# UnaryPlus/raytrace

Measured on AMD Instinct MI355X. Metric: Msamples/s (pixels×spp/s) + achieved HBM GB/s, Cornell-box 600×600, higher is better.
Workload: dtype f64; 1 GPU; cornell 600x600 200spp depth 50; width=600, height=600, spp=200, max_depth=50, parallelism=rows interleaved over 1 GPU(s), row_block 1

## Files before the change

raytrace_amd/csrc/rt_api.hip:

```cpp
#include <hip/hip_runtime.h>

#include <algorithm>
#include <chrono>
#include <cstdarg>
#include <cstdio>
#include <cstdlib>
#include <cstring>
#include <memory>
#include <mutex>
#include <string>
#include <thread>
#include <vector>

#include "../../include/rt.h"
#include "rt_denoise.h"
#include "rt_film.h"
#include "rt_internal.h"
#include "rt_kernel_class.h"

namespace {

thread_local std::string g_err;

int fail(int code, const char* fmt, ...) __attribute__((format(printf, 2, 3)));
// ... 200 lines not shown
  auto t0 = Clock::now();
  HIP_TRY(hipSetDevice(s->device));
  DevArrays<R>& A = s->arrays<R>();
  int rc = A.upload(s->host->arrays<R>(), s->nodes, s->perlin_perm);
  if (rc) {
    A.release();
    A = DevArrays<R>();
    return rc;
  }
  A.lds_nodes = 0;
  if ((s->variant & RT_VAR_BASE) != RT_VAR_FLAT) {
    const KernelClass c = rt_class_of(sizeof(R) == 8, s->variant);
    const int waves = std::max(1, rt_class_waves(sizeof(R) == 8, c));
    const int block = rt_class_block(sizeof(R) == 8, c);
    const int per_cu = std::max(1, 4 * waves * 64 / block);
    const int budget = (163840 / per_cu / 1024) * 1024 - 1024;
    const int used = (int)rt_class_lds_bytes(sizeof(R) == 8, c, s->stack_depth, 0);
    A.lds_nodes = std::max(0, std::min(s->host->surface_nodes, (budget - used) / 64));
    if (const char* e = rt_knob("RT_AMD_LDS_NODES")) A.lds_nodes = std::min(A.lds_nodes, std::max(0, atoi(e)));
  }
  A.resident_blocks = rt_render_resident_blocks((const KernelParamsT<R>*)nullptr, s->device, s->stack_depth,
                                                s->variant, A.lds_nodes);
  if (A.resident_blocks <= 0) {
    A.release();
    A = DevArrays<R>();
    return fail(RT_E_HIP, "occupancy query failed");
  }
  s->have<R>() = true;
  s->upload_ms += ms_since(t0);
  return RT_OK;
}

struct RenderCall {
  void* d_out = nullptr;
  char* ws = nullptr;
  size_t ws_cap = 0;
  int frame_rows = 0;
  bool lone = false, resolve = true;
  int sample0 = 0;
};

template <class R>
int render_async(const rt_device_scene* s, const rt_camera_settings* cs, uint64_t seed, const rt_exec* ex,
                 const RenderCall& c, void* hip_stream) {
  if (int rc = ensure_precision<R>(s)) return rc;
  const DevArrays<R>& A = s->arrays<R>();
  constexpr bool f64 = sizeof(R) == 8;
  LaunchInputs L;
  L.resident_lanes = (long long)A.resident_blocks * rt_class_block(f64, rt_class_of(f64, s->variant));
  L.lds_nodes = A.lds_nodes;
  L.lone = c.lone || (ex && (ex->flags & RT_EXEC_SOLO));
  L.sample0 = c.sample0;
  L.out_frame_rows = c.frame_rows;
  if (const char* e = rt_knob("RT_AMD_POOL_SHIFT")) L.pool_shift = std::max(4, std::min(10, atoi(e)));
  KernelParamsT<R> P;
  std::string err;
  int rc = rt_host_render_params(*s->host, s->variant, A.rec, cs, seed, ex, L, P, err);
  if (rc) return fail(rc, "%s", err.c_str());
  P.status = s->status;
  P.out = (R*)c.d_out;
  HIP_TRY(hipSetDevice(s->device));
  const Workspace W = workspace_layout((size_t)P.tile_rows * P.cam.width, RT_ACC_WORDS(R));
  hipStream_t st = (hipStream_t)hip_stream;
  char* ws = c.ws && c.ws_cap >= W.bytes ? c.ws : nullptr;
  const bool own = ws == nullptr;
  if (own) HIP_TRY(hipMallocAsync((void**)&ws, W.bytes, st));
  HIP_TRY(hipMemsetAsync(ws, 0, W.bytes, st));
  P.accum = (unsigned long long*)ws;
  P.nanflag = (unsigned int*)(ws + W.off_flag);
  P.counter = (int*)(ws + W.off_ctr);
  rc = RT_OK;
  int reserve = A.resident_blocks > 16 * RT_GRID_RESERVE ? RT_GRID_RESERVE : 0;
  if (const char* e = rt_knob("RT_AMD_GRID_RESERVE")) reserve = std::max(0, std::min(A.resident_blocks - 1, atoi(e)));
  if (rt_launch_render(P, A.resident_blocks - reserve, s->variant, hip_stream) ||
      (c.resolve && rt_launch_resolve(P, hip_stream)))
    rc = fail(RT_E_HIP, "kernel launch failed: %s", hipGetErrorString(hipGetLastError()));
  if (own) HIP_TRY(hipFreeAsync(ws, st));
  return rc;
}

int render_any(const rt_device_scene* s, const rt_camera_settings* cs, uint64_t seed, const rt_exec* ex, bool f32,
               const RenderCall& c, void* hip_stream) {
  return f32 ? render_async<float>(s, cs, seed, ex, c, hip_stream) : render_async<double>(s, cs, seed, ex, c, hip_stream);
}

int check_flags(const rt_exec* ex) {
  const int known = RT_EXEC_F32 | RT_EXEC_ENCODE8_SRGB | RT_EXEC_ENCODE8_SQRT | RT_EXEC_SOLO;
  if (ex->flags & ~known) return fail(RT_E_INVALID, "unknown rt_exec.flags bits 0x%x", ex->flags & ~known);
  if ((ex->flags & RT_EXEC_ENCODE8_SRGB) && (ex->flags & RT_EXEC_ENCODE8_SQRT))
    return fail(RT_E_INVALID, "rt_exec.flags: RT_EXEC_ENCODE8_SRGB and RT_EXEC_ENCODE8_SQRT are exclusive");
  return RT_OK;
}

int validate_frame(const rt_camera_settings* cs, uint64_t seed, const rt_exec* ex) {
  const int h = rt_host_image_height(cs);
  if (h <= 0 || cs->image_width <= 0) return fail(RT_E_INVALID, "image %dx%d must be non-empty", cs->image_width, h);
  if (rt_host_shard_rows(h, ex) < 0) return fail(RT_E_INVALID, "invalid rt_exec");
  if (int rc = check_flags(ex)) return rc;
  KernelParams P;
  std::string err;
  if (int rc = rt_host_make_params(cs, seed, ex, P, err)) return fail(rc, "%s", err.c_str());
  return RT_OK;
}

int exec_encoding(const rt_exec* ex) {
  if (!ex) return -1;
// ... 1136 lines not shown
```

raytrace_amd/csrc/rt_build.cpp:

```cpp
#include <algorithm>
#include <cmath>
#include <cstdarg>
#include <cstdio>
#include <cstdlib>
#include <cstring>
#include <optional>
#include <utility>

#include "../../include/rt.h"
#include "rt_bvh.h"
#include "rt_encode8_table.h"
#include "rt_internal.h"
#include "rt_kernel_class.h"

const char* rt_knob(const char* name) {
  const char* on = std::getenv("RT_AMD_EXPERIMENTS");
  if (!on || !*on || std::atoi(on) == 0) return nullptr;
  return std::getenv(name);
}

namespace {

struct d3 {
  double x, y, z;
// ... 1035 lines not shown
  const DevTargetT<R>& T = P.targets[0];
  for (int k = S.first; k < S.end_quad; ++k) {
    const R* f = A.flat_recs.data() + 16 * (size_t)k;
    if (std::memcmp(f, T.n, 3 * sizeof(R)) || std::memcmp(f + 4, T.q, 3 * sizeof(R)) ||
        std::memcmp(f + 8, T.wa, 3 * sizeof(R)) || std::memcmp(f + 12, T.wb, 3 * sizeof(R)))
      continue;
    int kf, slot;
    std::memcpy(&kf, f + 3, 4);
    std::memcpy(&slot, f + 11, 4);
    if (kf != 1 || slot < 0 || slot >= (int)A.prim_shade.size()) continue;
    if (A.prim_shade[slot].kind >= 2) continue;
    P.target_defer = 1;
    P.target_rec = k;
    return 1;
  }
  return 0;
}

template <class R>
SceneRecordsT<R> rt_host_records(const HostScene& H) {
  const HostArraysT<R>& A = H.arrays<R>();
  SceneRecordsT<R> r;
  r.nodes = H.nodes.data(), r.perlin_perm = H.perlin_perm.data();
  r.prims = A.prims.data(), r.prim_uv = A.prim_uv.data(), r.motions = A.motions.data();
  r.uvframes = A.uvframes.data(), r.texels = A.texels.data(), r.perlin_grad = A.perlin_grad.data();
  r.flat_recs = A.flat_recs.data(), r.prim_shade = A.prim_shade.data(), r.mats = A.mats.data();
  r.texs = A.texs.data(), r.boxes = A.boxes.data(), r.instances = A.instances.data();
  return r;
}

template <class R>
int rt_host_render_params(const HostScene& H, int variant, const SceneRecordsT<R>& r, const rt_camera_settings* cs,
                          uint64_t seed, const rt_exec* ex, const LaunchInputs& L, KernelParamsT<R>& P,
                          std::string& err) {
  constexpr bool f64 = sizeof(R) == 8;
  const bool flat = (variant & RT_VAR_BASE) == RT_VAR_FLAT;
  std::memset(&P, 0, sizeof P);
  if (int rc = rt_host_make_params(cs, seed, ex, P, err)) return rc;
  P.nodes = r.nodes, P.perlin_perm = r.perlin_perm;
  P.prims = r.prims, P.prim_uv = r.prim_uv, P.motions = r.motions, P.uvframes = r.uvframes, P.texels = r.texels;
  P.perlin_grad = r.perlin_grad, P.flat_recs = r.flat_recs, P.prim_shade = r.prim_shade, P.mats = r.mats;
  P.texs = r.texs, P.boxes = r.boxes, P.instances = r.instances;
  P.surface_root = H.surface_root;
  P.leaf_exit_pct = f64 ? H.leaf_exit_pct64 : H.leaf_exit_pct;
  P.surface_prefix = !flat && H.n_nodes > 0 ? 1 : 0;
  P.n_media = H.n_media;
  for (int k = 0; k < H.n_media; ++k) P.media[k] = H.arrays<R>().media[k];
  for (int k = 0; k <= RT_MAX_MEDIA; ++k) P.flat_sets[k] = H.flat_sets[k];
  P.stack_depth = rt_host_stack_depth(H);
  P.lds_nodes = L.lds_nodes;
  P.n_prims = H.n_prims;
  P.pool_shift = L.pool_shift ? L.pool_shift : L.lone && flat ? 6 : 0;
  rt_host_plan_work(P, L.resident_lanes, flat, L.lone);
  P.trav_exit_pct = f64 ? H.trav_exit_pct64 : H.trav_exit_pct;
  P.out_frame_rows = L.out_frame_rows;
  P.sample0 = L.sample0;
  rt_host_match_target(H, variant, P);
  return RT_OK;
}
#define RT_INSTANTIATE(R)                                                                                           \
  template int rt_host_match_target<R>(const HostScene&, int, KernelParamsT<R>&);                                   \
  template SceneRecordsT<R> rt_host_records<R>(const HostScene&);                                                   \
  template int rt_host_render_params<R>(const HostScene&, int, const SceneRecordsT<R>&, const rt_camera_settings*, \
                                        uint64_t, const rt_exec*, const LaunchInputs&, KernelParamsT<R>&, std::string&);
RT_INSTANTIATE(float)
RT_INSTANTIATE(double)
#undef RT_INSTANTIATE

bool rt_host_media_late(const HostScene& H) {
  if (H.n_media == 0) return false;
  for (int m = 0; m < H.n_media; ++m) {
    const DevMediumT<double>& M = H.f64.media[m];
    if (!M.alias_surface && !(M.root < 0 && M.root != RT_EMPTY_ROOT)) return false;
  }
  return true;
}

FastDiv rt_host_fastdiv(uint32_t d) {
  FastDiv f{0u, 0, d, 0};
  if (d <= 1) return f;
  int l = 0;
  while ((1ull << l) < d) ++l;
  f.m = (uint32_t)((((1ull << 32) * ((1ull << l) - d)) / d) + 1);
  f.s = l - 1;
  return f;
}

template <class R>
void rt_host_plan_work(KernelParamsT<R>& P, long long resident_lanes, bool two_sizes, bool lone) {
  P.div_width = rt_host_fastdiv((uint32_t)P.cam.width);
  P.div_block = rt_host_fastdiv((uint32_t)P.row_block);
  const bool pool_given = P.pool_shift >= 4;
  if (!pool_given) P.pool_shift = __builtin_ctz(RT_POOL);
  P.trav_exit_pct = 50;
  const long long tile_pixels = (long long)P.tile_rows * P.cam.width;
  const int spp = P.cam.spp;
  const int small = two_sizes ? 3 : 4;
  int chunk = spp < small ? spp : small;
  if (resident_lanes > 0 && (long long)P.tile_rows * P.cam.width * spp / 16 >= 64 * resident_lanes) chunk = 16;
  if (const char* env = rt_knob("RT_AMD_CHUNK")) {
    int c = std::atoi(env);
    if (c > 0) chunk = c;
  }
  int big = lone ? RT_BIG_CHUNK_MAX : RT_BIG_CHUNK_MAX_ASYNC, n_big = 0;
  if (const char* env = rt_knob("RT_AMD_BIG_CHUNK")) big = std::max(1, std::atoi(env));
  int tail_items = !lone ? RT_TAIL_ITEMS_ASYNC : sizeof(R) == 8 ? RT_TAIL_ITEMS_F64 : RT_TAIL_ITEMS_F32;
  if (const char* env = rt_knob("RT_AMD_TAIL_ITEMS")) tail_items = std::atoi(env);
  if (two_sizes && chunk < big && tail_items > 0 && resident_lanes > 0 && tile_pixels > 0) {
    long long t = ((long long)tail_items * chunk * resident_lanes + tile_pixels - 1) / tile_pixels;
    if (const char* env = rt_knob("RT_AMD_TAIL_SAMPLES")) t = std::max(0, std::atoi(env));
    const long long tail = ((t + chunk - 1) / chunk) * chunk;
    if (tail < spp) {
      const long long bulk = spp - tail;
      auto split = [&](int cap) {
        n_big = (int)((bulk + cap - 1) / cap);
        big = (int)((bulk + n_big - 1) / n_big);
        big = std::min(big, spp / n_big);
      };
      split(big);
      const double per_lane = (double)spp * (double)tile_pixels / (double)resident_lanes;
      for (int pass = 0; pass < 2 && !lone; ++pass) {
        const int pool_items = (pool_given ? 1 << P.pool_shift : big >= 32 ? 64 : RT_POOL) / 64;
        const int cap = (int)(0.9 * per_lane / pool_items);
        if (cap >= 1 && big > cap) split(cap);
      }
      if (big <= chunk) n_big = 0;
    }
  }
  const int n_chunks = (spp - n_big * big + chunk - 1) / chunk;
  long long items = (long long)(n_big + n_chunks) * tile_pixels;
  if (items > 0x7fffff00LL) {
    n_big = 0;
    chunk = (int)((long long)spp * tile_pixels / 0x7fffff00LL) + 1;
    items = (long long)((spp + chunk - 1) / chunk) * tile_pixels;
  }
  P.chunk = chunk;
  P.n_chunks = (spp - n_big * big + chunk - 1) / chunk;
  P.big_chunk = big;
  P.n_big_chunks = n_big;
  P.big_items = (int)((long long)n_big * tile_pixels);
  P.small_start = n_big * big;
  if (!pool_given && !lone && n_big > 0 && big >= 32) P.pool_shift = 6;
  P.div_big = rt_host_fastdiv((uint32_t)std::max(1, n_big));
  P.div_small = rt_host_fastdiv((uint32_t)std::max(1, P.n_chunks));
  P.n_items = (int)items;
  const KernelClass c{two_sizes ? RT_VAR_FLAT : RT_VAR_BVH, 0, P.n_media > 0 ? 1 : 0, false, false, 0, false};
  const int slot_pix = rt_class_agg_pix(sizeof(R) == 8, c);
  const int pool = 1 << P.pool_shift;
  auto spans = [&](int n) { return n > 0 && (pool - 1 + n - 1) / n + 1 <= slot_pix; };
  bool agg = tile_pixels < (1ll << 24);
  if (const char* env = rt_knob("RT_AMD_AGG")) agg = agg && std::atoi(env) != 0;
  P.agg_big = agg && spans(n_big);
  P.agg_small = agg && spans(P.n_chunks);
}

template int rt_host_make_params<float>(const rt_camera_settings*, uint64_t, const rt_exec*, KernelParamsT<float>&,
                                        std::string&);
template int rt_host_make_params<double>(const rt_camera_settings*, uint64_t, const rt_exec*, KernelParamsT<double>&,
                                         std::string&);
template void rt_host_plan_work<float>(KernelParamsT<float>&, long long, bool, bool);
template void rt_host_plan_work<double>(KernelParamsT<double>&, long long, bool, bool);

void rt_host_encode8_thresholds(int encoding, double* thr) {
  const double* t = encoding == 1 ? kEnc8Sqrt : kEnc8Srgb;
  for (int k = 0; k < 256; ++k) thr[k] = t[k];
}
```

raytrace_amd/csrc/rt_internal.h:

```cpp
#pragma once
#include <stdint.h>

#include <string>
#include <vector>

#ifndef RT_BLOCK
#define RT_BLOCK 64
#endif
#ifndef RT_BLOCK_BVH
#define RT_BLOCK_BVH 256
#endif
#define RT_MAX_NODES (1 << 26)
#define RT_STACK_DEPTH 64
#define RT_MAX_MEDIA 8
#define RT_MAX_TARGETS 8
#ifndef RT_LEAF_MAX
#define RT_LEAF_MAX 8
#endif
#ifndef RT_POOL
#define RT_POOL 128
#endif
#ifndef RT_AGG_SLOTS_FLAT
#define RT_AGG_SLOTS_FLAT 8
#endif
#ifndef RT_AGG_PIX_FLAT
#define RT_AGG_PIX_FLAT 17
#endif
#ifndef RT_AGG_SLOTS_FLAT_F64
#define RT_AGG_SLOTS_FLAT_F64 7
#endif
#ifndef RT_AGG_PIX_FLAT_F64
#define RT_AGG_PIX_FLAT_F64 22
#endif
#ifndef RT_AGG_SLOTS_BVH
#define RT_AGG_SLOTS_BVH 4
#endif
#ifndef RT_AGG_PIX_BVH
#define RT_AGG_PIX_BVH 5
#endif
#ifndef RT_BIG_CHUNK_MAX
#define RT_BIG_CHUNK_MAX 16
#endif
#ifndef RT_BIG_CHUNK_MAX_ASYNC
#define RT_BIG_CHUNK_MAX_ASYNC 64
#endif
#ifndef RT_TAIL_ITEMS_F64
#define RT_TAIL_ITEMS_F64 16
#endif
#ifndef RT_TAIL_ITEMS_F32
#define RT_TAIL_ITEMS_F32 32
#endif
#ifndef RT_TAIL_ITEMS_ASYNC
#define RT_TAIL_ITEMS_ASYNC 8
#endif
#define RT_LEAF_SHIFT 6
#define RT_FLAT_MAX 32
#define RT_LDS_PRIMS_MAX 256
#define RT_PREFIX_MAX 16
#ifndef RT_PREFIX_AREA
#define RT_PREFIX_AREA 0.1
#endif
#ifndef RT_PREFIX_SHRINK
#define RT_PREFIX_SHRINK 0.25
#endif
#define RT_EMPTY_ROOT ((int)0x80000000)
#ifndef RT_GRID_RESERVE
#define RT_GRID_RESERVE 0
#endif
#define RT_INST_FLAG 0x40000000
#define RT_INST_EXIT 0x7FFFFFFF

#define RT_VAR_FLAT 0
#define RT_VAR_BVH_LOCKSTEP 1
#ifndef RT_LOCKSTEP_KERNELS
#define RT_LOCKSTEP_KERNELS 0
#endif
#define RT_VAR_BVH 2
#define RT_VAR_BASE 3
#define RT_VAR_NOISE 4
#define RT_VAR_MEDIA 8
#define RT_VAR_MATS 16
#define RT_VAR_TEX 32
#define RT_VAR_INST 64
#define RT_VAR_LEAF_TRI 128
#define RT_VAR_LEAF_SPHERE 256
#define RT_VAR_MEDIA_LATE 512
#define RT_VAR_NARROW 1024
#define RT_WIDE_STACK_ROWS 23
const char* rt_knob(const char* name);

#define RT_KIND_MASK 3
#define RT_FLAG_MOTION 4
// ... 95 lines not shown
template <class R>
struct KernelParamsT {
  const float* nodes;
  const R* prims;
  const DevMaterialT<R>* prim_shade;
  const R* prim_uv;
  const DevMaterialT<R>* mats;
  const DevTextureT<R>* texs;
  const R* motions;
  const R* uvframes;
  const R* texels;
  const int* perlin_perm;
  const R* perlin_grad;
  const R* flat_recs;
  const DevBoxT<R>* boxes;
  const DevInstanceT<R>* instances;
  R* out;
  int* status;
  unsigned long long* accum;
  unsigned int* nanflag;
  int* counter;
  int chunk;
  int n_chunks;
  int n_items;
  int big_chunk;
  int n_big_chunks;
  int big_items;
  int small_start;
  FastDiv div_big, div_small;
  int agg_big, agg_small;
  int pool_shift;
  int stack_depth;
  int lds_nodes;
  int trav_exit_pct;
  int leaf_exit_pct;
  int n_prims;
  int surface_root;
  int surface_prefix;
  int n_media;
  int n_targets;
  R rem_prob;
  DevMediumT<R> media[RT_MAX_MEDIA];
  DevFlatSet flat_sets[1 + RT_MAX_MEDIA];
  DevTargetT<R> targets[RT_MAX_TARGETS];
  DevCameraT<R> cam;
  uint32_t key0, key1;
  int n_shards, shard, row_block, tile_rows;
  int out_frame_rows;
  FastDiv div_width, div_block;
  int sample0;
  int target_defer;
  int target_rec;
  int cam_defocus;
};
using DevMaterial = DevMaterialT<float>;
using DevTexture = DevTextureT<float>;
using DevMedium = DevMediumT<float>;
using DevBox = DevBoxT<float>;
using DevTarget = DevTargetT<float>;
using DevCamera = DevCameraT<float>;
using DevInstance = DevInstanceT<float>;
using KernelParams = KernelParamsT<float>;
using KernelParams64 = KernelParamsT<double>;

#define RT_FIX_SCALE 4294967296.0
#define RT_ACC_WORDS(R) (sizeof(R) == 8 ? 6 : 3)

template <class R>
struct HostArraysT {
  std::vector<R> prims, prim_uv, motions, uvframes, texels, perlin_grad;
  std::vector<R> flat_recs;
  std::vector<DevMaterialT<R>> prim_shade, mats;
  std::vector<DevTextureT<R>> texs;
  std::vector<DevBoxT<R>> boxes;
  std::vector<DevInstanceT<R>> instances;
  DevMediumT<R> media[RT_MAX_MEDIA];
};
struct HostScene {
  std::vector<float> nodes;
  std::vector<int> perlin_perm;
  std::vector<int> prim_mat;
  HostArraysT<float> f32;
  HostArraysT<double> f64;
  int surface_root = RT_EMPTY_ROOT;
  int n_media = 0;
  DevFlatSet flat_sets[1 + RT_MAX_MEDIA] = {};
  int n_nodes = 0, n_prims = 0, max_depth = 0, n_boxes = 0;
  int surface_nodes = 0;
  bool flat = false;
  bool noise = false;
  bool uv_tex = false;
  int leaf_exit_pct = 100;
  int leaf_exit_pct64 = 100;
  int trav_exit_pct = 50;
  int trav_exit_pct64 = 50;
  bool full_mats = false;
  int n_instances = 0;
  int leaf_kind = 0;
  template <class R>
  const HostArraysT<R>& arrays() const;
};
template <>
inline const HostArraysT<float>& HostScene::arrays<float>() const { return f32; }
template <>
inline const HostArraysT<double>& HostScene::arrays<double>() const { return f64; }

struct rt_scene;
struct rt_camera_settings;
struct rt_exec;

int rt_host_build_scene(const rt_scene* sc, HostScene& out, std::string& err);
int rt_host_image_height(const rt_camera_settings* cs);
int rt_host_shard_rows(int height, const rt_exec* ex);
bool rt_host_media_late(const HostScene& H);
int rt_host_variant(const HostScene& H);
int rt_host_variant(bool flat, int n_media, bool noise, bool mats, bool tex, bool inst, int leaf_kind, bool media_late,
                    int stack_depth);
inline int rt_host_stack_depth(const HostScene& H) { return H.max_depth > 1 ? H.max_depth : 1; }
template <class R>
int rt_host_make_params(const rt_camera_settings* cs, uint64_t seed, const rt_exec* ex, KernelParamsT<R>& P,
                        std::string& err);
template <class R>
struct SceneRecordsT {
  const float* nodes = nullptr;
  const int* perlin_perm = nullptr;
  const R *prims = nullptr, *prim_uv = nullptr, *motions = nullptr, *uvframes = nullptr, *texels = nullptr;
  const R *perlin_grad = nullptr, *flat_recs = nullptr;
  const DevMaterialT<R>*prim_shade = nullptr, *mats = nullptr;
  const DevTextureT<R>* texs = nullptr;
  const DevBoxT<R>* boxes = nullptr;
  const DevInstanceT<R>* instances = nullptr;
};
template <class R>
SceneRecordsT<R> rt_host_records(const HostScene& H);
struct LaunchInputs {
  long long resident_lanes = 0;
  int lds_nodes = 0;
  bool lone = false;
  int sample0 = 0, out_frame_rows = 0;
  int pool_shift = 0;
};
template <class R>
int rt_host_render_params(const HostScene& H, int variant, const SceneRecordsT<R>& records,
                          const rt_camera_settings* cs, uint64_t seed, const rt_exec* ex, const LaunchInputs& L,
                          KernelParamsT<R>& P, std::string& err);
template <class R>
int rt_host_match_target(const HostScene& H, int variant, KernelParamsT<R>& P);
template <class R>
void rt_host_plan_work(KernelParamsT<R>& P, long long resident_lanes, bool two_sizes, bool lone = false);
FastDiv rt_host_fastdiv(uint32_t d);
void rt_host_encode8_thresholds(int encoding, double* thr);

int rt_render_resident_blocks(const KernelParams*, int device, int stack_depth, int variant, int lds_nodes);
int rt_render_resident_blocks(const KernelParams64*, int device, int stack_depth, int variant, int lds_nodes);
int rt_launch_render(const KernelParams& p, int grid_blocks, int variant, void* stream);
int rt_launch_render(const KernelParams64& p, int grid_blocks, int variant, void* stream);
int rt_launch_resolve(const KernelParams& p, void* stream);
int rt_launch_resolve(const KernelParams64& p, void* stream);
int rt_launch_features(const KernelParams& p, int variant, unsigned long long* feat, int n_feat, void* stream);
int rt_launch_features(const KernelParams64& p, int variant, unsigned long long* feat, int n_feat, void* stream);
#if defined(RT_PHASE_PROF)
int rt_prof_read_kernel(const KernelParams*, unsigned long long* out, int n);
int rt_prof_read_kernel(const KernelParams64*, unsigned long long* out, int n);
#endif
#if defined(RT_WAVE_STAMPS)
int rt_stamps_read_kernel(const KernelParams*, unsigned long long* out, int n_waves);
int rt_stamps_read_kernel(const KernelParams64*, unsigned long long* out, int n_waves);
#endif
int rt_launch_encode8(const void* in, int in_f64, uint8_t* out, int64_t n, const double* thr, int encoding,
                      void* stream);
```

raytrace_amd/csrc/rt_kernel_class.h:

```cpp
#pragma once
#include <stddef.h>
#include <type_traits>
#include "rt_internal.h"

struct KernelClass {
  int var, tex, media; bool mats, inst; int leaf; bool narrow;
};

#ifndef RT_WAVES_FLAT
#define RT_WAVES_FLAT 7
#endif
#ifndef RT_WAVES_FLAT_NOISE
#define RT_WAVES_FLAT_NOISE 5
#endif
#ifndef RT_WAVES_BVH
#define RT_WAVES_BVH 5
#endif
#ifndef RT_WAVES_FLAT_TEX0
#define RT_WAVES_FLAT_TEX0 8
#endif
#ifndef RT_WAVES_BVH_LITE
#define RT_WAVES_BVH_LITE 6
#endif
#ifndef RT_WAVES64_FLAT_LITE
// ... 39 lines not shown
    if (c.inst && (!tex0 || c.media)) return RT_WAVES64_BVH_MEDIA;
    if (c.inst && c.mats) return RT_WAVES64_BVH_INST_MATS;
    if (c.media) return c.media == 2 ? RT_WAVES64_BVH_MEDIA_LATE : RT_WAVES64_BVH_MEDIA;
    if (tex0 && !c.mats) return RT_WAVES64_BVH_LITE;
    return tex0 && !c.inst ? RT_WAVES64_BVH_MATS : RT_WAVES64_BVH;
  }
  if (c.var == RT_VAR_FLAT) return c.tex == 2 ? RT_WAVES_FLAT_NOISE : tex0 ? RT_WAVES_FLAT_TEX0 : RT_WAVES_FLAT;
  if (c.media == 2) return c.inst ? RT_WAVES_BVH : RT_WAVES_BVH_MEDIA_LATE;
  if (c.media == 1 && c.inst) return RT_WAVES_BVH_INST_CHAIN;
  if (tex0 && !c.media && c.mats && !c.inst) return c.leaf == 0 ? RT_WAVES_BVH_MATS_GENERIC : RT_WAVES_BVH_MATS;
  return tex0 && !c.media ? RT_WAVES_BVH_LITE : RT_WAVES_BVH;
}

#ifndef RT_BIG_WG
#define RT_BIG_WG 1
#endif
constexpr int rt_class_block_wide(bool f64, KernelClass c) {
  if (c.var == RT_VAR_FLAT) return RT_BLOCK;
  const int w = rt_class_waves(f64, c);
  return RT_BIG_WG && (w == 3 || w == 6) ? 768 : RT_BIG_WG && (w == 4 || w == 8) ? 1024 : RT_BLOCK_BVH;
}
constexpr bool rt_class_has_twin(bool f64, KernelClass c) { return rt_class_block_wide(f64, c) == 1024; }
constexpr int rt_class_block(bool f64, KernelClass c) { return c.narrow ? 512 : rt_class_block_wide(f64, c); }

#ifndef RT_ACC_IN_LDS
#define RT_ACC_IN_LDS 1
#endif
constexpr bool rt_class_acc_lds(bool f64, KernelClass c) {
  return RT_ACC_IN_LDS && c.var != RT_VAR_FLAT && (f64 || !c.media);
}

constexpr bool rt_class_agg_wide(bool f64, KernelClass c) { return f64 || c.media == 0; }
constexpr int rt_class_agg_slots(bool f64, KernelClass c) {
  return c.var != RT_VAR_FLAT ? RT_AGG_SLOTS_BVH : rt_class_agg_wide(f64, c) ? RT_AGG_SLOTS_FLAT_F64 : RT_AGG_SLOTS_FLAT;
}
constexpr int rt_class_agg_pix(bool f64, KernelClass c) {
  return c.var != RT_VAR_FLAT ? RT_AGG_PIX_BVH : rt_class_agg_wide(f64, c) ? RT_AGG_PIX_FLAT_F64 : RT_AGG_PIX_FLAT;
}
static_assert(RT_AGG_SLOTS_FLAT < 255 && RT_AGG_SLOTS_FLAT_F64 < 255 && RT_AGG_SLOTS_BVH < 255,
              "slot + 1 must fit the 8 bits of rt_trace.h ItemCtx::tp");
constexpr int rt_acc_words(bool f64) { return f64 ? RT_ACC_WORDS(double) : RT_ACC_WORDS(float); }
constexpr int rt_class_agg_bytes(bool f64, KernelClass c) {
  return rt_class_agg_slots(f64, c) * (rt_class_agg_pix(f64, c) * rt_acc_words(f64) * 8 + 2 * 4);
}
constexpr size_t rt_class_fixed_lds(bool f64, KernelClass c) {
  const size_t block = (size_t)rt_class_block(f64, c);
  return (rt_class_acc_lds(f64, c) ? rt_acc_words(f64) * 8 * block : 0) + rt_class_agg_bytes(f64, c) * (block / 64);
}
constexpr size_t rt_class_lds_bytes(bool f64, KernelClass c, int stack_depth, int lds_nodes) {
  return rt_class_fixed_lds(f64, c) +
         (c.var == RT_VAR_FLAT ? 0 : (size_t)(stack_depth + 1) * rt_class_block(f64, c) * sizeof(int) + (size_t)lds_nodes * 64);
}

#ifndef RT_NOLICM_FLAT_LITE
#define RT_NOLICM_FLAT_LITE 0
#endif
#ifndef RT_NOLICM_BVH_LITE
#define RT_NOLICM_BVH_LITE 0
#endif
constexpr bool rt_class_nolicm(bool f64, KernelClass c) {
  const bool heavy = c.tex != 0 || c.media != 0 || c.mats;
  return c.var == RT_VAR_FLAT ? f64 && (RT_NOLICM_FLAT_LITE || heavy) : RT_NOLICM_BVH_LITE || heavy || c.inst;
}

#ifndef RT_LEAF_MEDIA
#define RT_LEAF_MEDIA 1
#endif
constexpr bool rt_media_late_compiled(int var) { return var == RT_VAR_BVH; }
constexpr bool rt_leaf_compiled(int var, int tex, int media, bool inst, int leaf) {
  if (leaf == 0) return true;
  if (var != RT_VAR_BVH || inst) return false;
  return media ? RT_LEAF_MEDIA && tex == 0 && leaf == 1 : true;
}
constexpr bool rt_class_compiled(bool f64, KernelClass c) {
  if (c.var == RT_VAR_BVH_LOCKSTEP && !RT_LOCKSTEP_KERNELS) return false;
  if (c.var != RT_VAR_BVH && c.inst) return false;
  if (c.media == 2 && !rt_media_late_compiled(c.var)) return false;
  return rt_leaf_compiled(c.var, c.tex, c.media, c.inst, c.leaf) && (!c.narrow || rt_class_has_twin(f64, c));
}

constexpr KernelClass rt_class_of(bool f64, int variant) {
  const int base = variant & RT_VAR_BASE;
  KernelClass c{};
  c.inst = (variant & RT_VAR_INST) != 0;
  c.var = c.inst || (base == RT_VAR_BVH_LOCKSTEP && !RT_LOCKSTEP_KERNELS) ? RT_VAR_BVH : base;
  c.tex = (variant & RT_VAR_NOISE) ? 2 : (variant & RT_VAR_TEX) ? 1 : 0;
  c.media = !(variant & RT_VAR_MEDIA) ? 0 : (variant & RT_VAR_MEDIA_LATE) && rt_media_late_compiled(base) ? 2 : 1;
  c.mats = (variant & RT_VAR_MATS) != 0;
  const int leaf = (variant & RT_VAR_LEAF_TRI) ? 1 : (variant & RT_VAR_LEAF_SPHERE) ? 2 : 0;
  c.leaf = rt_leaf_compiled(base, c.tex, c.media, c.inst, leaf) ? leaf : 0;
  c.narrow = (variant & RT_VAR_NARROW) && rt_class_has_twin(f64, c);
  return c;
}

constexpr bool rt_every_class(bool (*p)(bool, KernelClass)) {
  for (int v = 0; v < 2 * RT_VAR_NARROW; ++v)
    if ((v & RT_VAR_BASE) != RT_VAR_BASE && !(p(false, rt_class_of(false, v)) && p(true, rt_class_of(true, v))))
      return false;
  return true;
}
static_assert(rt_every_class(rt_class_compiled), "rt_class_of names a class that is not compiled");
constexpr bool rt_wide_rows_fit(bool f64, KernelClass c) {
  return !rt_class_has_twin(f64, c) || rt_class_lds_bytes(f64, c, RT_WIDE_STACK_ROWS - 1, 0) <= 163840 - 1024;
}
static_assert(rt_every_class(rt_wide_rows_fit), "RT_WIDE_STACK_ROWS stack rows must fit a 1024-lane workgroup's LDS");

// ... 14 lines not shown
```

raytrace_amd/csrc/rt_render_kernel.h:

```cpp
#include <hip/hip_runtime.h>
#include <stdint.h>

#include <type_traits>

#include "rt_kernel_class.h"
#include "rt_trace.h"

namespace RT_NS {

#if defined(RT_WAVE_STAMPS)
#define RT_STAMP_WAVES 16384
static __device__ unsigned long long rt_stamp_buf[4 * RT_STAMP_WAVES];
#endif

namespace {

static_assert(RT_POOL >= 64, "a refill must cover every lane of a wave");
#ifndef RT_QUEUES
#define RT_QUEUES 4
#endif
#ifndef RT_QUEUE_INTERLEAVE
#define RT_QUEUE_INTERLEAVE 1
#endif
static_assert((RT_QUEUES & (RT_QUEUES - 1)) == 0 && RT_QUEUES <= 8, "RT_QUEUES: a power of two, at most 8 (workspace)");
// ... 117 lines not shown
      }
      first += take;
      rest -= take;
      pool_base = qs + base + take;
      pool_left = avail - take;
      if (rest > 0) {
        queue = (queue + 1) & (RT_QUEUES - 1);
        ++spent;
      }
    }
    return item;
  }

  __device__ __forceinline__ void direct(int tp, const Acc& A) const {
    unsigned long long* a = kp().accum + RT_ACC_WORDS(real) * (size_t)tp;
#pragma unroll
    for (int c = 0; c < 3; ++c)
      if (A.hi[c]) atomicAdd(a + c, (unsigned long long)A.hi[c]);
#if RT_F64
#pragma unroll
    for (int c = 0; c < 3; ++c)
      if (A.lo[c]) atomicAdd(a + 3 + c, A.lo[c]);
#endif
  }
  __device__ __forceinline__ bool aggregating() const { return kSlots > 0 && (kp().agg_big | kp().agg_small) != 0; }
  __device__ __forceinline__ int untag(int tpk) const { return aggregating() ? (tpk & 0xffffff) : tpk; }
  __device__ __forceinline__ int tag(int tp, int slot) const {
    if (slot < 0) return tp;
    return tp | ((slot + 1) << 24);
  }
  template <class AccT>
  __device__ __forceinline__ void commit(bool c, int tpk, const AccT& acc, bool bad) {
    if (!c) return;
    const int code = aggregating() ? (int)((uint32_t)tpk >> 24) : 0;
    const int tp = code ? tpk & 0xffffff : tpk;
    const Acc A = acc_words(acc);
    if (code == 0) {
      direct(tp, A);
    } else {
      const int s = code - 1;
      unsigned long long* w = slots + s * AggGeom<kSlots, kPix>::kWords + (tp - hdr[kSlots + s]) * RT_ACC_WORDS(real);
#pragma unroll
      for (int k = 0; k < 3; ++k)
        if (A.hi[k]) lds_add(w + k, (unsigned long long)A.hi[k]);
#if RT_F64
#pragma unroll
      for (int k = 0; k < 3; ++k)
        if (A.lo[k]) lds_add(w + 3 + k, A.lo[k]);
#endif
      __hip_atomic_fetch_add(hdr + s, -1, __ATOMIC_RELAXED, __HIP_MEMORY_SCOPE_WORKGROUP);
    }
    if (bad) atomicOr(kp().nanflag + tp, 1u);
  }
  __device__ __forceinline__ void flush(int s) {
    constexpr int kW = AggGeom<kSlots, kPix>::kWords;
    const unsigned long long act = __ballot(true);
    const int k = (int)__popcll(act);
    const int r = (int)__popcll(act & ((1ull << __lane_id()) - 1ull));
    const int tplo = __builtin_amdgcn_readfirstlane(hdr[kSlots + s]);
    const long long g0 = (long long)tplo * RT_ACC_WORDS(real);
    const long long g_end = (long long)kp().tile_rows * kp().cam.width * RT_ACC_WORDS(real);
    unsigned long long* w = slots + s * kW;
    for (int j = r; j < kW; j += k) {
      const unsigned long long v = w[j];
      if (v != 0ull) {
        w[j] = 0ull;
        if (g0 + j < g_end) atomicAdd(kp().accum + g0 + j, v);
      }
    }
    free_mask |= 1u << s;
  }
};

}

#ifndef RT_TU_NOLICM
#define RT_TU_NOLICM 0
#endif
template <int kVar, int kTex, int kMedia, bool kMats, bool kInst, int kLeaf, bool kNarrow = false>
__global__ __launch_bounds__(rt_class_block(RT_F64, KernelClass{kVar, kTex, kMedia, kMats, kInst, kLeaf, kNarrow}))
__attribute__((amdgpu_waves_per_eu(rt_class_waves(RT_F64, KernelClass{kVar, kTex, kMedia, kMats, kInst, kLeaf, kNarrow}))))
void rt_render_kernel(KernelParams P) {
  extern __shared__ int smem[];
#if defined(RT_WAVE_STAMPS)
  const unsigned long long t_start = wall_clock64();
#endif
  constexpr KernelClass kC{kVar, kTex, kMedia, kMats, kInst, kLeaf, kNarrow};
  constexpr int kSlots = rt_class_agg_slots(RT_F64, kC), kPix = rt_class_agg_pix(RT_F64, kC);
#if defined(RT_BLOCK_RUNTIME)
  const int block = (int)blockDim.x;
#else
  constexpr int block = rt_class_block(RT_F64, kC);
#endif
#if defined(RT_BLOCK_RUNTIME_STACK)
  const int block_stack = (int)blockDim.x;
#else
  const int block_stack = block;
#endif
#if defined(RT_BLOCK_RUNTIME_NODES)
  const int block_nodes = (int)blockDim.x;
#else
  const int block_nodes = block;
#endif
#if defined(RT_BLOCK_RUNTIME_COPY)
  const int block_copy = (int)blockDim.x;
#else
// ... 1 lines not shown
#endif
  constexpr int kAggBytes = rt_class_agg_bytes(RT_F64, kC);
  const int waves = (int)(gridDim.x * (blockDim.x / 64));
  const int wave_in_block = __builtin_amdgcn_readfirstlane((int)(threadIdx.x / 64));
  const int wave = (int)blockIdx.x * (int)(blockDim.x / 64) + wave_in_block;
  int overflow;
  using AccT = typename std::conditional<rt_class_acc_lds(RT_F64, kC), AccLds, Acc>::type;
  AccT acc;
  int* smem_rest = smem;
  if constexpr (rt_class_acc_lds(RT_F64, kC)) {
    acc = AccLds{reinterpret_cast<unsigned long long*>(smem) + threadIdx.x, (int)blockDim.x};
    smem_rest = smem + 2 * RT_ACC_WORDS(real) * (int)blockDim.x;
  }
  unsigned long long* agg = reinterpret_cast<unsigned long long*>(smem_rest) + kAggBytes / 8 * wave_in_block;
  smem_rest += kAggBytes / 4 * (int)(blockDim.x / 64);
  for (int i = (int)__lane_id(); i < kAggBytes / 8; i += 64) agg[i] = 0ull;
#if defined(RT_WAVE_STAMPS)
#define RT_STAMP_END(work)                                                                        \
  if (__lane_id() == 0 && wave < RT_STAMP_WAVES) {                                                \
    rt_stamp_buf[4 * wave] = t_start;                                                             \
    rt_stamp_buf[4 * wave + 1] = work.t_drain;                                                    \
    rt_stamp_buf[4 * wave + 2] = wall_clock64();                                                  \
    rt_stamp_buf[4 * wave + 3] = (unsigned long long)__builtin_amdgcn_s_getreg((4 << 0) | (31 << 11)) << 32 | \
                                 (unsigned)__builtin_amdgcn_s_getreg((20 << 0) | (3 << 11));      \
  }
#else
#define RT_STAMP_END(work)
#endif
  if constexpr (kVar == RT_VAR_FLAT) {
    WaveWork<kSlots, kPix, true> work(P, wave, waves, agg);
    overflow = lane_loop_lockstep<true, kTex, kMedia != 0, kMats>(P, work, Trav{nullptr, 0, nullptr}, P.prims, acc);
    work.finish();
    RT_STAMP_END(work)
  } else {
    v4f* lds_nodes = reinterpret_cast<v4f*>(smem_rest + (P.stack_depth + 1) * block_nodes);
    const float4* src = reinterpret_cast<const float4*>(P.nodes);
    for (int i = threadIdx.x; i < 4 * P.lds_nodes; i += block_copy) {
      const float4 q = src[i];
      lds_nodes[i] = v4f{q.x, q.y, q.z, q.w};
    }
    __syncthreads();
    WaveWork<kSlots, kPix, RT_KARGS_WORK_BVH> work(P, wave, waves, agg);
    const Trav W{smem_rest + threadIdx.x, block_stack, lds_nodes};
    if constexpr (kVar == RT_VAR_BVH_LOCKSTEP)
      overflow = lane_loop_lockstep<false, kTex, kMedia != 0, kMats>(P, work, W, P.prims, acc);
    else
      overflow = lane_loop_bvh<kTex, kMedia, kMats, kInst, kLeaf>(P, work, W, P.prims, acc);
    work.finish();
    RT_STAMP_END(work)
  }
  if (overflow) atomicOr(P.status, 1);
}

#ifndef RT_KERNEL_ONLY
#if !RT_TU_NOLICM
__global__ __launch_bounds__(256) void rt_resolve_kernel(const long long* __restrict__ accum,
                                                         const unsigned int* __restrict__ nanflag,
                                                         real* __restrict__ out, int n_pixels, int spp, double scale,
                                                         int width, int frame_rows, int n_shards, int shard,
                                                         int row_block) {
  const int i = blockIdx.x * 256 + threadIdx.x;
  if (i >= n_pixels) return;
  size_t w = 3 * (size_t)i + blockIdx.y;
  if (frame_rows > 0) {
    const int t = i / width, px = i - t * width;
    const int g = ((t / row_block) * n_shards + shard) * row_block + t % row_block;
    if (g >= frame_rows) return;
    w = 3 * ((size_t)g * width + px) + blockIdx.y;
  }
  const bool bad = nanflag[i] != 0u;
#if RT_F64
  (void)scale;
  const long long* a = accum + 6 * (size_t)i + blockIdx.y;
  const double sum = ((double)a[0] + (double)(unsigned long long)a[3] * (1.0 / RT_FIX_SCALE)) * (1.0 / RT_FIX_SCALE);
  out[w] = bad ? __builtin_nan("") : sum / (double)spp;
#else
  (void)spp;
  out[w] = bad ? __builtin_nanf("") : (float)((double)accum[3 * (size_t)i + blockIdx.y] * scale);
#endif
}
#endif

typedef void (*render_fn)(KernelParams);
static render_fn render_kernel_this_tu(int variant) {
  return rt_with_class(rt_class_of(RT_F64, variant), [](auto... k) -> render_fn {
    constexpr KernelClass c{decltype(k)::value...};
    if constexpr (rt_class_compiled(RT_F64, c) && rt_class_nolicm(RT_F64, c) == (bool)RT_TU_NOLICM)
      return rt_render_kernel<c.var, c.tex, c.media, c.mats, c.inst, c.leaf, c.narrow>;
    return nullptr;
  });
}
render_fn render_kernel_nolicm(int variant);
template <class T, size_t N>
static int diag_read(T (&buf)[N], unsigned long long* out, size_t n) {
  if (hipMemcpyFromSymbol(out, HIP_SYMBOL(buf), n * sizeof(T)) != hipSuccess) return -1;
  void* p = nullptr;
  if (hipGetSymbolAddress(&p, HIP_SYMBOL(buf)) != hipSuccess) return -1;
  return hipMemset(p, 0, sizeof(buf)) == hipSuccess ? 0 : -1;
}
int diag_read_nolicm(int which, unsigned long long* out, size_t n);
static int diag_read_this_tu(int which, unsigned long long* out, size_t n) {
  (void)which, (void)out, (void)n;
#if defined(RT_PHASE_PROF)
  if (which == 0) return diag_read(rt_prof_buf, out, n);
#endif
#if defined(RT_WAVE_STAMPS)
  if (which == 1) return diag_read(rt_stamp_buf, out, n);
#endif
  return -1;
}
#if RT_TU_NOLICM
int diag_read_nolicm(int which, unsigned long long* out, size_t n) { return diag_read_this_tu(which, out, n); }
#endif
static int diag_read_both(int which, unsigned long long* out, size_t n) {
  if (hipDeviceSynchronize() != hipSuccess || diag_read_this_tu(which, out, n)) return -1;
  unsigned long long* other = new unsigned long long[n];
  const int rc = diag_read_nolicm(which, other, n);
  for (size_t k = 0; k < n && rc == 0; ++k) out[k] += other[k];
  delete[] other;
  return rc;
}
#if RT_TU_NOLICM
render_fn render_kernel_nolicm(int variant) { return render_kernel_this_tu(variant); }
#else
static render_fn render_kernel_of(int variant) {
  const render_fn f = render_kernel_this_tu(variant);
  return f ? f : render_kernel_nolicm(variant);
}
#endif

#endif
}
#if !defined(RT_KERNEL_ONLY) && !RT_TU_NOLICM

int rt_render_resident_blocks(const KernelParamsT<RT_NS::real>*, int device, int stack_depth, int variant,
                              int lds_nodes) {
  using namespace RT_NS;
  int per_cu = 0, cus = 0;
  const KernelClass c = rt_class_of(RT_F64, variant);
  size_t lds = rt_class_lds_bytes(RT_F64, c, stack_depth, lds_nodes);
  if (lds > 65536 && hipFuncSetAttribute((const void*)render_kernel_of(variant),
                                         hipFuncAttributeMaxDynamicSharedMemorySize, (int)lds) != hipSuccess)
    return -1;
  hipError_t e =
      hipOccupancyMaxActiveBlocksPerMultiprocessor(&per_cu, render_kernel_of(variant), rt_class_block(RT_F64, c), lds);
  if (e != hipSuccess) return -1;
  if (hipDeviceGetAttribute(&cus, hipDeviceAttributeMultiprocessorCount, device) != hipSuccess) return -1;
  if (per_cu < 1) per_cu = 1;
  return per_cu * cus;
}

int rt_launch_render(const KernelParamsT<RT_NS::real>& p, int grid_blocks, int variant, void* stream) {
  using namespace RT_NS;
  if (p.n_items <= 0 || grid_blocks <= 0) return 0;
  const KernelClass c = rt_class_of(RT_F64, variant);
  const int block = rt_class_block(RT_F64, c);
  long long need = ((long long)p.n_items + block - 1) / block;
  int grid = need < grid_blocks ? (int)need : grid_blocks;
  size_t lds = rt_class_lds_bytes(RT_F64, c, p.stack_depth, p.lds_nodes);
  hipLaunchKernelGGL(render_kernel_of(variant), dim3(grid), dim3(block), lds, (hipStream_t)stream, p);
  return hipGetLastError() == hipSuccess ? 0 : -1;
}

#if defined(RT_PHASE_PROF)
int rt_prof_read_kernel(const KernelParamsT<RT_NS::real>*, unsigned long long* out, int n) {
  using namespace RT_NS;
  if (n > PF_N) n = PF_N;
  return diag_read_both(0, out, (size_t)n) == 0 ? n : -1;
}
#endif

#if defined(RT_WAVE_STAMPS)
int rt_stamps_read_kernel(const KernelParamsT<RT_NS::real>*, unsigned long long* out, int n_waves) {
  using namespace RT_NS;
  if (n_waves > RT_STAMP_WAVES) n_waves = RT_STAMP_WAVES;
  return diag_read_both(1, out, 4 * (size_t)n_waves) == 0 ? n_waves : -1;
}
#endif

int rt_launch_resolve(const KernelParamsT<RT_NS::real>& p, void* stream) {
  using namespace RT_NS;
  int n = p.tile_rows * p.cam.width;
  if (n <= 0) return 0;
  hipLaunchKernelGGL(rt_resolve_kernel, dim3((n + 255) / 256, 3), dim3(256), 0, (hipStream_t)stream,
                     (const long long*)p.accum, p.nanflag, p.out, n, p.cam.spp, 1.0 / (RT_FIX_SCALE * (double)p.cam.spp),
                     p.cam.width, p.out_frame_rows, p.n_shards, p.shard, p.row_block);
  return hipGetLastError() == hipSuccess ? 0 : -1;
}
#endif
```

raytrace_amd/csrc/rt_trace.h:

```cpp
#ifndef RT_TRACE_COMMON_H
#define RT_TRACE_COMMON_H
#include <stdint.h>

#include "../../include/rt.h"
#include "rt_internal.h"
#include "rt_sincos_table.h"

#ifdef RT_HOST_EMU
#include <cmath>
#include <cstring>
#define RT_FN static inline
#define RT_FN_SPEC inline
namespace rt_emu {
inline int f2i(float f) {
  int i;
  std::memcpy(&i, &f, 4);
  return i;
}
extern thread_local long long counters[4];
}
#define RT_F2I(f) rt_emu::f2i(f)
#define RT_COUNT(i) (++rt_emu::counters[i])
#define RT_ANY(x) (x)
#define RT_BALLOT_COUNT(x) ((x) ? 1 : 0)
// ... 1588 lines not shown
    } else {
      closest<kFlat>(P, prims, P.surface_root, 0, R, kTmin, C, TW, &overflow);
    }
    real tbest = C.t;
    const int best = C.prim;
    int hit_medium = -1;
    const int n_media = kMedia ? P.n_media : 0;
    for (int m = 0; m < n_media; ++m) {
      const DevMedium& M = P.media[m];
      Closest C1 = no_hit();
      if (M.alias_surface) {
        C1.t = C.t;
        C1.prim = C.prim;
      } else {
        closest<kFlat>(P, prims, M.root, m + 1, R, kTmin, C1, TW, &overflow);
      }
      if (C1.prim < 0) continue;
      const real t1 = C1.t;
      real lo, hi;
      if (prim_front(P, prims, C1.prim, R, t1)) {
        if (!(t1 < tbest)) continue;
        Closest C2 = no_hit();
        closest<kFlat>(P, prims, M.root, m + 1, R, t1, C2, TW, &overflow);
        if (C2.prim < 0) continue;
        lo = t1;
        hi = C2.t;
      } else {
        lo = kTmin;
        hi = t1;
      }
      medium_event(P, m, I.pix, I.sample, seg, lo, hi, tbest, hit_medium);
    }
    RT_PROF_MARK(PF_TRAV);
    f3 L = mk3(RL(0.), RL(0.), RL(0.));
    bool ended;
    if constexpr (kDefer)
      ended = shade<kTex, kMats, false>(P, prims, I.pix, I.sample, seg, tbest, best, hit_medium, R, L, T, -1, &apdf);
    else
      ended = shade<kTex, kMats>(P, prims, I.pix, I.sample, seg, tbest, best, hit_medium, R, L, T);
    if (ended) {
#ifdef RT_HOST_EMU
      apdf = RT_NAN;
#endif
      RT_HOOK_SAMPLE(I.pix, I.sample, L);
      acc_sample(acc, L, bad);
      alive = false;
      ++I.sample;
    }
    RT_PROF_MARK(PF_SHADE);
  }
  RT_PROF_FLUSH
  return overflow;
}

template <bool kInst>
RT_FN void media_events_late(const KernelParams& P, cfp prims, const RayCtx& R, uint32_t pix, int sample, int seg, int best,
                             real t_surf, real& tbest, int& hit_medium) {
  for (int m = 0; m < P.n_media; ++m) {
    const DevMedium& M = P.media[m];
    bool ev = false;
    real lo = kTmin, hi = t_surf;
    if (M.alias_surface) {
      ev = best >= 0 && !prim_front(P, prims, best, R, t_surf);
    } else {
      const int enc = ~M.root;
      const int first = enc >> RT_LEAF_SHIFT, end = first + (enc & ((1 << RT_LEAF_SHIFT) - 1)) + 1;
      Closest C1 = no_hit();
      for (int k = first; k < end; ++k)
        test_rec<false, kInst>(P, ld_rec64((const RT_CAS PrimRec64*)prims + k), k, R, kTmin, float_up(kTmin), C1);
      if (C1.prim >= 0) {
        const real t1 = C1.t;
        if (prim_front(P, prims, C1.prim, R, t1)) {
          if (t1 < tbest) {
            Closest C2 = no_hit();
            for (int k = first; k < end; ++k)
              test_rec<false, kInst>(P, ld_rec64((const RT_CAS PrimRec64*)prims + k), k, R, t1, float_up(t1), C2);
            ev = C2.prim >= 0;
            lo = t1;
            hi = C2.t;
          }
        } else {
          ev = true;
          hi = t1;
        }
      }
    }
    if (ev) medium_event(P, m, pix, sample, seg, lo, hi, tbest, hit_medium);
  }
}

enum : int { ST_NEED_ITEM = 0, ST_NEED_SAMPLE = 1, ST_START_SEG = 2, ST_TRACE = 3, ST_SHADE = 4 };
template <int kTex, int kMedia, bool kMats, bool kInst, int kLeaf, class Work, class AccT>
RT_FN int lane_loop_bvh(const KernelParams& P0, Work& work, const Trav& TW, const real* prims_, AccT& acc) {
  const cfp prims = cf(prims_);
  const int n_media = kMedia == 1 ? P0.n_media : 0;
  int overflow = 0;
  ItemCtx I{-1, 0, 0, 0u, 0u};
  int seg = 0;
  acc_clear(acc);
  bool bad = false;
  int state = ST_NEED_ITEM;
  f3 T = mk3(RL(1.), RL(1.), RL(1.));
  RayCtx R;
  R.o = R.d = mk3(RL(0.), RL(0.), RL(0.));
#if RT_NODE_F32
  R.idir = R.off0 = R.off1 = f3n{0.f, 0.f, 0.f};
// ... 151 lines not shown
```

Baseline: 16570 Msamples/s.

## Add wave-level camera-ray ring kernel for flat scenes with per-sample work items

Adds a new flat-scene render kernel where each work item is a single (pixel, sample). Wave lanes that finish a path refill from an LDS ring of pre-generated camera rays, which are produced cooperatively by the whole wave when the ring runs low. This keeps lanes busy and cuts divergence from uneven path lengths, and it comes with a new pool-size heuristic and a per-slot LDS aggregation for accumulating samples. The cost is extra LDS traffic and ballot/prefix overhead, plus more atomics per sample than the chunked scheme. It is enabled by default for eligible flat classes.

```diff
diff --git a/raytrace_amd/csrc/rt_api.hip b/raytrace_amd/csrc/rt_api.hip
--- a/raytrace_amd/csrc/rt_api.hip
+++ b/raytrace_amd/csrc/rt_api.hip
@@ -276,6 +276,7 @@
   L.lone = c.lone || (ex && (ex->flags & RT_EXEC_SOLO));
   L.sample0 = c.sample0;
   L.out_frame_rows = c.frame_rows;
+  L.flat_ring = true;
   if (const char* e = rt_knob("RT_AMD_POOL_SHIFT")) L.pool_shift = std::max(4, std::min(10, atoi(e)));
   KernelParamsT<R> P;
   std::string err;
diff --git a/raytrace_amd/csrc/rt_build.cpp b/raytrace_amd/csrc/rt_build.cpp
--- a/raytrace_amd/csrc/rt_build.cpp
+++ b/raytrace_amd/csrc/rt_build.cpp
@@ -1111,6 +1111,7 @@
   P.n_prims = H.n_prims;
   P.pool_shift = L.pool_shift ? L.pool_shift : L.lone && flat ? 6 : 0;
   rt_host_plan_work(P, L.resident_lanes, flat, L.lone);
+  if (L.flat_ring) rt_host_plan_ring(P, variant, L.lone, L.pool_shift, L.resident_lanes);
   P.trav_exit_pct = f64 ? H.trav_exit_pct64 : H.trav_exit_pct;
   P.out_frame_rows = L.out_frame_rows;
   P.sample0 = L.sample0;
@@ -1213,6 +1214,41 @@
   P.agg_small = agg && spans(P.n_chunks);
 }
 
+template <class R>
+bool rt_host_plan_ring(KernelParamsT<R>& P, int variant, bool lone, int pool_shift, long long resident_lanes) {
+  P.flat_ring = 0;
+  if (!rt_class_has_ring(rt_class_of(sizeof(R) == 8, variant))) return false;
+  if (const char* e = rt_knob("RT_AMD_FLAT_RING"))
+    if (std::atoi(e) == 0) return false;
+  const long long tile_pixels = (long long)P.tile_rows * P.cam.width;
+  const int spp = P.cam.spp;
+  if (spp <= 0 || tile_pixels <= 0 || tile_pixels * spp > 0x7fffff00LL) return false;
+  const bool pool_given = pool_shift >= 4;
+  int shift = pool_given ? pool_shift : lone ? 9 : 10;
+  auto spans = [&](int s) { return ((1 << s) - 1 + spp - 1) / spp + 1 <= RT_RING_AGG_PIX; };
+  const long long waves = resident_lanes / 64;
+  auto spreads = [&](int s) { return waves <= 0 || (8ll << s) * waves <= tile_pixels * spp; };
+  while (!pool_given && shift > 6 && !(spans(shift) && spreads(shift))) --shift;
+  P.pool_shift = shift;
+  P.chunk = 1;
+  P.n_chunks = spp;
+  P.big_chunk = 1;
+  P.n_big_chunks = 0;
+  P.big_items = 0;
+  P.small_start = 0;
+  P.div_big = rt_host_fastdiv(1u);
+  P.div_small = rt_host_fastdiv((uint32_t)spp);
+  P.n_items = (int)(tile_pixels * spp);
+  bool agg = tile_pixels < (1ll << 24);
+  if (const char* env = rt_knob("RT_AMD_AGG")) agg = agg && std::atoi(env) != 0;
+  P.agg_big = 0;
+  P.agg_small = agg && spans(shift);
+  P.flat_ring = 1;
+  return true;
+}
+template bool rt_host_plan_ring<float>(KernelParamsT<float>&, int, bool, int, long long);
+template bool rt_host_plan_ring<double>(KernelParamsT<double>&, int, bool, int, long long);
+
 template int rt_host_make_params<float>(const rt_camera_settings*, uint64_t, const rt_exec*, KernelParamsT<float>&,
                                         std::string&);
 template int rt_host_make_params<double>(const rt_camera_settings*, uint64_t, const rt_exec*, KernelParamsT<double>&,
diff --git a/raytrace_amd/csrc/rt_internal.h b/raytrace_amd/csrc/rt_internal.h
--- a/raytrace_amd/csrc/rt_internal.h
+++ b/raytrace_amd/csrc/rt_internal.h
@@ -38,6 +38,10 @@
 #ifndef RT_AGG_PIX_BVH
 #define RT_AGG_PIX_BVH 5
 #endif
+#define RT_RING_LANES 64
+#define RT_RING_AGG_PIX 8
+#define RT_RING_AGG_SLOTS_F64 6
+#define RT_RING_AGG_SLOTS_F32 5
 #ifndef RT_BIG_CHUNK_MAX
 #define RT_BIG_CHUNK_MAX 16
 #endif
@@ -239,6 +243,7 @@
   int target_defer;
   int target_rec;
   int cam_defocus;
+  int flat_ring;
 };
 using DevMaterial = DevMaterialT<float>;
 using DevTexture = DevTextureT<float>;
@@ -326,6 +331,7 @@
   bool lone = false;
   int sample0 = 0, out_frame_rows = 0;
   int pool_shift = 0;
+  bool flat_ring = false;
 };
 template <class R>
 int rt_host_render_params(const HostScene& H, int variant, const SceneRecordsT<R>& records,
@@ -335,6 +341,8 @@
 int rt_host_match_target(const HostScene& H, int variant, KernelParamsT<R>& P);
 template <class R>
 void rt_host_plan_work(KernelParamsT<R>& P, long long resident_lanes, bool two_sizes, bool lone = false);
+template <class R>
+bool rt_host_plan_ring(KernelParamsT<R>& P, int variant, bool lone, int pool_shift = 0, long long resident_lanes = 0);
 FastDiv rt_host_fastdiv(uint32_t d);
 void rt_host_encode8_thresholds(int encoding, double* thr);
 
diff --git a/raytrace_amd/csrc/rt_kernel_class.h b/raytrace_amd/csrc/rt_kernel_class.h
--- a/raytrace_amd/csrc/rt_kernel_class.h
+++ b/raytrace_amd/csrc/rt_kernel_class.h
@@ -115,6 +115,19 @@
          (c.var == RT_VAR_FLAT ? 0 : (size_t)(stack_depth + 1) * rt_class_block(f64, c) * sizeof(int) + (size_t)lds_nodes * 64);
 }
 
+constexpr KernelClass rt_ring_class() { return KernelClass{RT_VAR_FLAT, 0, 0, false, false, 0, false}; }
+constexpr bool rt_class_has_ring(KernelClass c) {
+  return c.var == RT_VAR_FLAT && c.tex == 0 && c.media == 0 && !c.mats && !c.inst;
+}
+constexpr int rt_ring_agg_slots(bool f64) { return f64 ? RT_RING_AGG_SLOTS_F64 : RT_RING_AGG_SLOTS_F32; }
+constexpr int rt_ring_agg_bytes(bool f64) { return rt_ring_agg_slots(f64) * (RT_RING_AGG_PIX * rt_acc_words(f64) * 8 + 2 * 4); }
+constexpr int rt_ring_ray_bytes(bool f64) { return RT_RING_LANES * (6 * (f64 ? 8 : 4) + 4 * 4); }
+constexpr size_t rt_ring_lds_bytes(bool f64) { return (size_t)rt_ring_ray_bytes(f64) + rt_ring_agg_bytes(f64); }
+static_assert(RT_BLOCK == RT_RING_LANES, "the ring belongs to a one-wave workgroup");
+static_assert(rt_ring_lds_bytes(false) <= rt_class_fixed_lds(false, rt_ring_class()) &&
+                  rt_ring_lds_bytes(true) <= rt_class_fixed_lds(true, rt_ring_class()),
+              "the ring form's LDS must not exceed the legacy kernel's (same workgroups per CU)");
+
 #ifndef RT_NOLICM_FLAT_LITE
 #define RT_NOLICM_FLAT_LITE 0
 #endif
diff --git a/raytrace_amd/csrc/rt_render_kernel.h b/raytrace_amd/csrc/rt_render_kernel.h
--- a/raytrace_amd/csrc/rt_render_kernel.h
+++ b/raytrace_amd/csrc/rt_render_kernel.h
@@ -193,6 +193,34 @@
     }
     if (bad) atomicOr(kp().nanflag + tp, 1u);
   }
+  __device__ __forceinline__ int tag_ring(int tp, int slot) const {
+    static_assert(kSlots <= 7 && kPix <= 32, "tag_ring: 3 bits of slot + 1, 5 bits of pixel offset");
+    if (slot < 0) return tp;
+    return (int)((uint32_t)tp | (uint32_t)((slot + 1) | ((tp - hdr[kSlots + slot]) << 3)) << 24);
+  }
+  __device__ __forceinline__ void skip_ring(bool c, int tpk) {
+    if (!c || !aggregating()) return;
+    const int code = (int)((uint32_t)tpk >> 24) & 7;
+    if (code) __hip_atomic_fetch_add(hdr + code - 1, -1, __ATOMIC_RELAXED, __HIP_MEMORY_SCOPE_WORKGROUP);
+  }
+  __device__ __forceinline__ void commit_ring(int tpk, const Acc& A, bool bad) {
+    const uint32_t code = aggregating() ? (uint32_t)tpk >> 24 : 0u;
+    const int tp = code ? tpk & 0xffffff : tpk;
+    if (code == 0u) {
+      direct(tp, A);
+    } else {
+      const int s = (int)(code & 7u) - 1;
+      unsigned long long* w = slots + s * AggGeom<kSlots, kPix>::kWords + (int)(code >> 3) * RT_ACC_WORDS(real);
+#pragma unroll
+      for (int k = 0; k < 3; ++k) lds_add(w + k, (unsigned long long)A.hi[k]);
+#if RT_F64
+#pragma unroll
+      for (int k = 0; k < 3; ++k) lds_add(w + 3 + k, A.lo[k]);
+#endif
+      __hip_atomic_fetch_add(hdr + s, -1, __ATOMIC_RELAXED, __HIP_MEMORY_SCOPE_WORKGROUP);
+    }
+    if (bad) atomicOr(kp().nanflag + tp, 1u);
+  }
   __device__ __forceinline__ void flush(int s) {
     constexpr int kW = AggGeom<kSlots, kPix>::kWords;
     const unsigned long long act = __ballot(true);
@@ -300,6 +328,21 @@
   if (overflow) atomicOr(P.status, 1);
 }
 
+#if !RT_TU_NOLICM
+__global__ __launch_bounds__(RT_BLOCK) __attribute__((amdgpu_waves_per_eu(rt_class_waves(RT_F64, rt_ring_class()))))
+void rt_render_kernel_ring(KernelParams P) {
+  extern __shared__ int smem[];
+  real* ring_od = reinterpret_cast<real*>(smem);
+  uint32_t* ring_meta = reinterpret_cast<uint32_t*>(ring_od + 6 * RT_RING_LANES);
+  unsigned long long* agg = reinterpret_cast<unsigned long long*>(ring_meta + 4 * RT_RING_LANES);
+  constexpr int kAggBytes = rt_ring_agg_bytes(RT_F64);
+  for (int i = (int)__lane_id(); i < kAggBytes / 8; i += 64) agg[i] = 0ull;
+  WaveWork<rt_ring_agg_slots(RT_F64), RT_RING_AGG_PIX, true> work(P, (int)blockIdx.x, (int)gridDim.x, agg);
+  lane_loop_flat_ring(P, work, ring_od, ring_meta);
+  work.finish();
+}
+#endif
+
 #ifndef RT_KERNEL_ONLY
 #if !RT_TU_NOLICM
 __global__ __launch_bounds__(256) void rt_resolve_kernel(const long long* __restrict__ accum,
@@ -405,6 +448,11 @@
   const int block = rt_class_block(RT_F64, c);
   long long need = ((long long)p.n_items + block - 1) / block;
   int grid = need < grid_blocks ? (int)need : grid_blocks;
+  if (p.flat_ring) {
+    if (!rt_class_has_ring(c)) return -1;
+    hipLaunchKernelGGL(rt_render_kernel_ring, dim3(grid), dim3(block), rt_ring_lds_bytes(RT_F64), (hipStream_t)stream, p);
+    return hipGetLastError() == hipSuccess ? 0 : -1;
+  }
   size_t lds = rt_class_lds_bytes(RT_F64, c, p.stack_depth, p.lds_nodes);
   hipLaunchKernelGGL(render_kernel_of(variant), dim3(grid), dim3(block), lds, (hipStream_t)stream, p);
   return hipGetLastError() == hipSuccess ? 0 : -1;
diff --git a/raytrace_amd/csrc/rt_trace.h b/raytrace_amd/csrc/rt_trace.h
--- a/raytrace_amd/csrc/rt_trace.h
+++ b/raytrace_amd/csrc/rt_trace.h
@@ -1664,6 +1664,106 @@
   RT_PROF_FLUSH
   return overflow;
 }
+
+#ifndef RT_HOST_EMU
+RT_FN int wave_prefix(unsigned long long m) {
+  return (int)__builtin_amdgcn_mbcnt_hi((uint32_t)(m >> 32), __builtin_amdgcn_mbcnt_lo((uint32_t)m, 0u));
+}
+template <class Work>
+RT_FN void lane_loop_flat_ring(const KernelParams& P0, Work& work, real* ring_od, uint32_t* ring_meta) {
+  constexpr int kN = RT_RING_LANES;
+  int cnt = 0;
+  bool drained = false;
+  bool alive = false;
+  uint32_t pix = 0u;
+  int sample = 0, tpk = 0, seg = 0;
+  f3 T = mk3(RL(1.), RL(1.), RL(1.));
+  real apdf = RL(1.);
+  RayCtx R;
+  R.o = R.d = mk3(RL(0.), RL(0.), RL(0.));
+#if RT_NODE_F32
+  R.idir = R.off0 = R.off1 = f3n{0.f, 0.f, 0.f};
+#else
+  R.idir = R.oidir = R.o;
+#endif
+  R.time_w = 0u;
+  R.self_gid = -1;
+  R.self_inst = -1;
+  RT_PROF_DECL
+  for (;;) {
+    const KernelParams& P = RT_KARGS(P0);
+    const bool need = !alive;
+    const unsigned long long m = __ballot(need);
+    RT_PROF_ADD(PF_ITERS, 1);
+    RT_PROF_ADD(PF_CAM_LANES, (int)__popcll(m));
+    if (m != 0ull) {
+      const int rank = wave_prefix(m);
+      int want = (int)__popcll(m), base = 0;
+      for (;;) {
+        const int take = want < cnt ? want : cnt;
+        const int k = rank - base;
+        if (need && k >= 0 && k < take) {
+          const int e = cnt - 1 - k;
+          R.o = mk3(ring_od[e], ring_od[kN + e], ring_od[2 * kN + e]);
+          R.d = mk3(ring_od[3 * kN + e], ring_od[4 * kN + e], ring_od[5 * kN + e]);
+          R.time_w = ring_meta[e];
+          pix = ring_meta[kN + e];
+          sample = (int)ring_meta[2 * kN + e];
+          tpk = (int)ring_meta[3 * kN + e];
+          R.self_gid = -1;
+          T = mk3(RL(1.), RL(1.), RL(1.));
+          seg = 0;
+          alive = true;
+        }
+        cnt -= take;
+        base += take;
+        want -= take;
+        if (want == 0 || drained) break;
+        RT_PROF_ADD(PF_FRONT_LANES, kN);
+        int aslot;
+        const int got = work.grab(true, aslot);
+        const bool in = got < P.n_items;
+        ItemCtx J{-1, 0, 0, 0u, 0u};
+        const bool ok = in && open_item<true>(P, got, J);
+        const int jt = work.tag_ring(J.tp, aslot);
+        work.skip_ring(in && !ok, jt);
+        const unsigned long long vm = __ballot(ok);
+        if (ok) {
+          RayCtx C;
+          camera_ray_flat(P, J.pix, J.sample, J.pxgy, C);
+          const int e = wave_prefix(vm);
+          ring_od[e] = C.o.x, ring_od[kN + e] = C.o.y, ring_od[2 * kN + e] = C.o.z;
+          ring_od[3 * kN + e] = C.d.x, ring_od[4 * kN + e] = C.d.y, ring_od[5 * kN + e] = C.d.z;
+          ring_meta[e] = C.time_w;
+          ring_meta[kN + e] = J.pix;
+          ring_meta[2 * kN + e] = (uint32_t)J.sample;
+          ring_meta[3 * kN + e] = (uint32_t)jt;
+        }
+        __builtin_amdgcn_wave_barrier();
+        cnt = (int)__popcll(vm);
+        drained = __ballot(in) != ~0ull;
+      }
+    }
+    RT_PROF_MARK(PF_FRONT);
+    if (!alive) break;
+    Closest C = no_hit();
+    closest_flat<true>(P, 0, R, kTmin, C, &apdf);
+    if (P.target_defer) T = (seg == 0 ? RL(1.) : RT_RCP(apdf)) * T;
+    RT_PROF_MARK(PF_TRAV);
+    f3 L = mk3(RL(0.), RL(0.), RL(0.));
+    if (shade<0, false, false>(P, cf(P.prims), pix, sample, seg, C.t, C.prim, -1, R, L, T, -1, &apdf)) {
+      Acc a;
+      acc_clear(a);
+      bool bad = false;
+      acc_sample(a, L, bad);
+      work.commit_ring(tpk, a, bad);
+      alive = false;
+    }
+    RT_PROF_MARK(PF_SHADE);
+  }
+  RT_PROF_FLUSH
+}
+#endif
 
 template <bool kInst>
 RT_FN void media_events_late(const KernelParams& P, cfp prims, const RayCtx& R, uint32_t pix, int sample, int seg, int best,
```

Result: faster. 17430 Msamples/s, median of 6 (+5.2%).
